# pfe-rs/lk-s-2022-estimacija-pokreta

Hardware: AMD Instinct MI355X
Metric: Mpix/s flow (1024x436, bcd_times=4) (higher is better)
Workload: dtype f64; 1 GPU; single 1024x436 Sintel-shape pair per step per GPU, forward only, bcd_times=4 (BASELINE.json configs[1]); cells 64x27, 150 labels/px; pairs_in_flight_per_gpu=7, mode=batch

## Files before the change

### include/dflow.h

```cpp
#ifndef DFLOW_H
#define DFLOW_H

#include <stddef.h>
#include <stdint.h>

#ifdef __cplusplus
extern "C" {
#endif

#define DFLOW_VERSION 1
#define DFLOW_DESC 68
#define DFLOW_MAX_LABELS 160

#define DFLOW_FLAG_KNN_EXACT 1

#define DFLOW_FLAG_DESCR_F16 8
#define DFLOW_DESC_PITCH_F16 72

#define DFLOW_OK 0
#define DFLOW_EINVAL (-1)
#define DFLOW_ENOSPC (-2)
#define DFLOW_EHIP (-3)

#define DFLOW_DP_SENTINEL 800000.0
// ... 4 lines not shown
    int32_t maxnprop;
    int32_t knn;
    int32_t window;
    int32_t ngauss;
    int32_t tpsi;
    int32_t max_attempts;
    float tphi;
    float sigma;
    double lamda;
    uint64_t seed;
    int32_t label_pitch;
    int32_t flags;
} dflow_params;

int dflow_version(void);
const char *dflow_last_error(void);

void dflow_default_params(dflow_params *p, int32_t pich, int32_t picw, int32_t cellh, int32_t cellw);

size_t dflow_workspace_bytes(const dflow_params *p);

int dflow_daisy(const dflow_params *p, const uint8_t *d_bgr, void *d_descr,
                void *d_ws, size_t ws_bytes, void *stream);

int dflow_knn_proposals(const dflow_params *p, const void *d_descr1, const void *d_descr2,
                        uint32_t *d_proposals, float *d_lcosts, int32_t *d_nprop, int32_t *d_bestlabels,
                        void *d_ws, size_t ws_bytes, void *stream);

int dflow_knn_proposals_timed(const dflow_params *p, const void *d_descr1, const void *d_descr2,
                              uint32_t *d_proposals, float *d_lcosts, int32_t *d_nprop, int32_t *d_bestlabels,
                              void *d_ws, size_t ws_bytes, void *stream, float *h_ms, double *h_mfma_issued);

#define DFLOW_KNN_STATS_N 13
int dflow_knn_screen_stats(const dflow_params *p, void *d_ws, size_t ws_bytes, void *stream, int64_t *h_stats);

#define DFLOW_KNN_STATS_ALL_N 14
int dflow_knn_screen_stats_n(const dflow_params *p, void *d_ws, size_t ws_bytes, void *stream, int64_t *h_stats, int n_stats);

int dflow_neighbour_proposals(const dflow_params *p, const void *d_descr1, const void *d_descr2,
                              uint32_t *d_proposals, float *d_lcosts, int32_t *d_nprop,
                              const int32_t *d_bestlabels, void *d_ws, size_t ws_bytes, void *stream);

int dflow_bcd_prepare(const dflow_params *p, const uint32_t *d_proposals, const float *d_lcosts, const int32_t *d_nprop,
                      void *d_ws, size_t ws_bytes, void *stream);

int dflow_bcd_phase(const dflow_params *p, const uint32_t *d_proposals, const int32_t *d_nprop,
// ... 74 lines not shown
```

### lk-s-2022-estimacija-pokreta_amd/_lib.py

```python
import ctypes as C
import os
import subprocess

_HERE = os.path.dirname(os.path.abspath(__file__))
CSRC = os.path.join(_HERE, "csrc")
LIB_PATH = os.path.join(CSRC, "libdflow.so")

FLAG_KNN_EXACT = 1
FLAG_DESCR_F16 = 8
DESC_PITCH_F16 = 72
VAR_FLAG_SOR_UNFUSED = 1
EVAL_UVV, EVAL_DYDX = 0, 1
EVAL_FLAG_ACCUMULATE = 1


class DflowError(RuntimeError):
    pass


class Params(C.Structure):
    _fields_ = [("pich", C.c_int32), ("picw", C.c_int32), ("cellh", C.c_int32), ("cellw", C.c_int32),
                ("maxnprop", C.c_int32), ("knn", C.c_int32), ("window", C.c_int32), ("ngauss", C.c_int32),
                ("tpsi", C.c_int32), ("max_attempts", C.c_int32), ("tphi", C.c_float), ("sigma", C.c_float),
                ("lamda", C.c_double), ("seed", C.c_uint64), ("label_pitch", C.c_int32), ("flags", C.c_int32)]


class VarParams(C.Structure):
    _fields_ = [("alpha", C.c_float), ("gamma", C.c_float), ("delta", C.c_float), ("sigma", C.c_float),
                ("sor_omega", C.c_float), ("niter_outer", C.c_int32), ("niter_inner", C.c_int32),
                ("niter_solver", C.c_int32), ("flags", C.c_uint32)]


class EvalStats(C.Structure):
    _fields_ = [("n", C.c_uint64), ("n_out_abs", C.c_uint64), ("n_out_kitti", C.c_uint64), ("n_nonfinite", C.c_uint64),
                ("n_gt_valid", C.c_uint64), ("n_test_valid", C.c_uint64), ("sum_err", C.c_double), ("max_err", C.c_float),
                ("reserved", C.c_uint32)]


_vp, _sz, _i32, _f32, _f64 = C.c_void_p, C.c_size_t, C.c_int32, C.c_float, C.c_double
_pp = C.POINTER(Params)
_SIGNATURES = {
    "dflow_version": (C.c_int, []),
    "dflow_last_error": (C.c_char_p, []),
    "dflow_default_params": (None, [_pp, _i32, _i32, _i32, _i32]),
    "dflow_workspace_bytes": (_sz, [_pp]),
    "dflow_daisy": (C.c_int, [_pp, _vp, _vp, _vp, _sz, _vp]),
    "dflow_knn_proposals": (C.c_int, [_pp, _vp, _vp, _vp, _vp, _vp, _vp, _vp, _sz, _vp]),
    "dflow_knn_proposals_timed": (C.c_int, [_pp, _vp, _vp, _vp, _vp, _vp, _vp, _vp, _sz, _vp, C.POINTER(_f32), C.POINTER(_f64)]),
    "dflow_knn_screen_stats": (C.c_int, [_pp, _vp, _sz, _vp, C.POINTER(C.c_int64)]),
    "dflow_knn_screen_stats_n": (C.c_int, [_pp, _vp, _sz, _vp, C.POINTER(C.c_int64), _i32]),
    "dflow_neighbour_proposals": (C.c_int, [_pp, _vp, _vp, _vp, _vp, _vp, _vp, _vp, _sz, _vp]),
    "dflow_bcd_prepare": (C.c_int, [_pp, _vp, _vp, _vp, _vp, _sz, _vp]),
    "dflow_bcd_phase": (C.c_int, [_pp, _vp, _vp, _vp, _i32, _vp, _sz, _vp]),
    "dflow_bcd_sweep": (C.c_int, [_pp, _vp, _vp, _vp, _vp, _sz, _vp]),
    "dflow_bcd_phase_batch": (C.c_int, [_pp, _i32, _vp, _vp, _i32, _vp, _sz, _vp]),
    "dflow_bcd_sweep_batch": (C.c_int, [_pp, _i32, _vp, _vp, _vp, _sz, _vp]),
    "dflow_labels_to_flow": (C.c_int, [_pp, _vp, _vp, _vp, _vp]),
    "dflow_fb_consistency": (C.c_int, [_pp, _vp, _vp, _f32, _vp, _vp]),
    "dflow_pack_compat": (C.c_int, [_pp, _vp, _vp, _vp, _vp]),
    "dflow_remove_small_segments_host": (C.c_int, [_vp, _i32, _i32, _f32, _i32]),
    "dflow_canny_workspace_bytes": (_sz, [_i32, _i32]),
    "dflow_canny_edges": (C.c_int, [_i32, _i32, _vp, _f64, _f64, _vp, _vp, _vp, _sz, _vp]),
    "dflow_pb_workspace_bytes": (_sz, [_i32, _i32]),
    "dflow_pb_edges": (C.c_int, [_i32, _i32, _vp, _i32, _vp, _vp, _vp, _sz, _vp]),
    "dflow_epic_workspace_bytes": (_sz, [_i32, _i32]),
    "dflow_epic_interpolate": (C.c_int, [_i32, _i32, _vp, _vp, _i32, _f64, _i32, _vp, _vp, _vp, _vp, _vp, _vp, _sz, _vp]),
    "dflow_epic_last_stats": (C.c_int, [_vp, _vp]),
    "dflow_epic_prefilter_workspace_bytes": (_sz, [_i32, _i32]),
    "dflow_epic_prefilter": (C.c_int, [_i32, _i32, _vp, _vp, _vp, _f64, _i32, _f64, _f64, _vp, _vp, _vp, _vp, _vp, _sz, _vp]),
# ... 67 lines not shown
```

### lk-s-2022-estimacija-pokreta_amd/csrc/abi.hip

```cpp
#include <math.h>
#include <stdarg.h>
#include <stdio.h>
#include <stdlib.h>
#include <string.h>
#include "dflow_common.h"

static thread_local char g_err[512] = "";

int dflow_set_error(int code, const char *fmt, ...)
{
    va_list ap;
    va_start(ap, fmt);
    vsnprintf(g_err, sizeof(g_err), fmt, ap);
    va_end(ap);
    return code;
}

int dflow_check_launch(const char *what)
{
    hipError_t e = hipGetLastError();
    if (e != hipSuccess) return dflow_set_error(DFLOW_EHIP, "%s: %s", what, hipGetErrorString(e));
    return DFLOW_OK;
}

// ... 26 lines not shown
    if (!(p->sigma > 0.0f) || p->sigma > 8.0f) return dflow_set_error(DFLOW_EINVAL, "sigma=%g outside (0,8]", (double)p->sigma);
    if (p->max_attempts < p->ngauss) return dflow_set_error(DFLOW_EINVAL, "max_attempts < ngauss");
    if (p->flags & ~(DFLOW_FLAG_KNN_EXACT | DFLOW_FLAG_DESCR_F16)) return dflow_set_error(DFLOW_EINVAL, "unknown flags 0x%x", (unsigned)p->flags);
    return DFLOW_OK;
}

extern "C" {

int dflow_version(void) { return DFLOW_VERSION; }

const char *dflow_last_error(void) { return g_err; }

void dflow_default_params(dflow_params *p, int32_t pich, int32_t picw, int32_t cellh, int32_t cellw)
{
    memset(p, 0, sizeof(*p));
    p->pich = pich; p->picw = picw; p->cellh = cellh; p->cellw = cellw;
    p->maxnprop = 150; p->knn = 5; p->window = 2; p->ngauss = 25; p->tpsi = 8; p->max_attempts = 1 << 16;
    p->tphi = 2.5f; p->sigma = 8.0f; p->lamda = 0.05; p->seed = 0; p->label_pitch = 160;
}

size_t dflow_workspace_bytes(const dflow_params *p)
{
    if (dflow_check_params(p) != DFLOW_OK) return 0;
    size_t m = daisy_ws_bytes(p);
    for (size_t b : {bcd_ws_bytes(p), neighbour_ws_bytes(p), knn_mfma_supported(p) ? knn_mfma_ws_bytes(p) : (size_t)0})
        if (b > m) m = b;
    return m + DFLOW_WS_SLACK;
}

#define CHECK_PTR(x) do { if (!(x)) return dflow_set_error(DFLOW_EINVAL, "%s: %s is NULL", __func__, #x); } while (0)
#define CHECK_WS(need) do { if (!d_ws || ws_bytes < (need)) \
    return dflow_set_error(DFLOW_ENOSPC, "%s: workspace %zu < %zu bytes", __func__, ws_bytes, (size_t)(need)); } while (0)

int dflow_daisy(const dflow_params *p, const uint8_t *d_bgr, void *d_descr, void *d_ws, size_t ws_bytes, void *stream)
{
    int rc = dflow_check_params(p); if (rc) return rc;
    CHECK_PTR(d_bgr); CHECK_PTR(d_descr); CHECK_WS(daisy_ws_bytes(p));
    return launch_daisy(p, d_bgr, d_descr, d_ws, (hipStream_t)stream);
}

int dflow_knn_proposals(const dflow_params *p, const void *d_descr1, const void *d_descr2, uint32_t *d_proposals,
                        float *d_lcosts, int32_t *d_nprop, int32_t *d_bestlabels, void *d_ws, size_t ws_bytes, void *stream)
{
    int rc = dflow_check_params(p); if (rc) return rc;
    CHECK_PTR(d_descr1); CHECK_PTR(d_descr2); CHECK_PTR(d_proposals); CHECK_PTR(d_lcosts); CHECK_PTR(d_nprop); CHECK_PTR(d_bestlabels);
    if ((p->flags & DFLOW_FLAG_KNN_EXACT) || !knn_mfma_supported(p))
        return launch_knn(p, d_descr1, d_descr2, d_proposals, d_lcosts, d_nprop, d_bestlabels, (hipStream_t)stream);
    CHECK_WS(knn_mfma_ws_bytes(p));
    return launch_knn_mfma(p, d_descr1, d_descr2, d_proposals, d_lcosts, d_nprop, d_bestlabels, d_ws, (hipStream_t)stream);
}

int dflow_knn_proposals_timed(const dflow_params *p, const void *d_descr1, const void *d_descr2, uint32_t *d_proposals,
                              float *d_lcosts, int32_t *d_nprop, int32_t *d_bestlabels, void *d_ws, size_t ws_bytes, void *stream,
                              float *h_ms, double *h_mfma_issued)
{
    int rc = dflow_check_params(p); if (rc) return rc;
    CHECK_PTR(d_descr1); CHECK_PTR(d_descr2); CHECK_PTR(d_proposals); CHECK_PTR(d_lcosts); CHECK_PTR(d_nprop); CHECK_PTR(d_bestlabels);
    CHECK_PTR(h_ms);
    if ((p->flags & DFLOW_FLAG_KNN_EXACT) || !knn_mfma_supported(p))
        return dflow_set_error(DFLOW_EINVAL, "%s: the MFMA-screened search does not run for these parameters", __func__);
    CHECK_WS(knn_mfma_ws_bytes(p));
// ... 281 lines not shown
```

### lk-s-2022-estimacija-pokreta_amd/csrc/daisy.hip

```cpp
#include <math.h>
#include "dflow_common.h"

#define MAX_TAPS 9
struct Taps { int n; float k[MAX_TAPS]; };

struct GridTab { double gy[17], gx[17]; };

__device__ static inline int clampi(int v, int lo, int hi) { return v < lo ? lo : (v > hi ? hi : v); }

__device__ static inline float gray_of(const uint8_t *__restrict__ bgr, int W, int y, int x)
{
    return (float)gray_u8(bgr, W, y, x) / 255.0f;
}

template <typename T> __device__ static inline T tmul(float k, T v);
template <> __device__ inline float tmul<float>(float k, float v) { return k * v; }
template <> __device__ inline float4 tmul<float4>(float k, float4 v) { return make_float4(k * v.x, k * v.y, k * v.z, k * v.w); }
__device__ static inline float tadd(float a, float b) { return a + b; }
__device__ static inline float4 tadd(float4 a, float4 b) { return make_float4(a.x + b.x, a.y + b.y, a.z + b.z, a.w + b.w); }

struct LayerW { float wc[4], ws[4]; };

#define FX 32
#define FY 8
__global__ void __launch_bounds__(FX * FY) front_kernel(const uint8_t *__restrict__ bgr, float4 *__restrict__ lay, int H, int W, Taps t, LayerW w)
{
    __shared__ float g[FY + 6][FX + 6], th[FY + 6][FX + 2], sm[FY + 2][FX + 2];
    const int gx0 = blockIdx.x * FX, gy0 = blockIdx.y * FY, tid = threadIdx.y * FX + threadIdx.x;
    for (int i = tid; i < (FY + 6) * (FX + 6); i += FX * FY) {
        const int r = i / (FX + 6), c = i % (FX + 6);
        g[r][c] = gray_of(bgr, W, clampi(gy0 - 3 + r, 0, H - 1), clampi(gx0 - 3 + c, 0, W - 1));
    }
    __syncthreads();
    for (int i = tid; i < (FY + 6) * (FX + 2); i += FX * FY) {
        const int r = i / (FX + 2), c = i % (FX + 2);
        const int X = clampi(gx0 - 1 + c, 0, W - 1);
        float acc = t.k[0] * g[r][clampi(X - 2, 0, W - 1) - (gx0 - 3)];
#pragma unroll
        for (int j = 1; j < 5; j++) acc = acc + t.k[j] * g[r][clampi(X - 2 + j, 0, W - 1) - (gx0 - 3)];
        th[r][c] = acc;
    }
    __syncthreads();
    for (int i = tid; i < (FY + 2) * (FX + 2); i += FX * FY) {
        const int r = i / (FX + 2), c = i % (FX + 2);
        const int Y = clampi(gy0 - 1 + r, 0, H - 1);
        float acc = t.k[0] * th[clampi(Y - 2, 0, H - 1) - (gy0 - 3)][c];
#pragma unroll
        for (int j = 1; j < 5; j++) acc = acc + t.k[j] * th[clampi(Y - 2 + j, 0, H - 1) - (gy0 - 3)][c];
        sm[r][c] = acc;
    }
    __syncthreads();
    const int x = gx0 + threadIdx.x, y = gy0 + threadIdx.y;
    if (x >= W || y >= H) return;
    const int c = threadIdx.x + 1, r = threadIdx.y + 1;
    const float dx = (sm[r][c + 1] - sm[r][c - 1]) * 0.5f;
    const float dy = (sm[r + 1][c] - sm[r - 1][c]) * 0.5f;
    float v[4];
#pragma unroll
    for (int l = 0; l < 4; l++) { float q = dx * w.wc[l] + dy * w.ws[l]; v[l] = q > 0.0f ? q : 0.0f; }
    lay[(size_t)y * W + x] = make_float4(v[0], v[1], v[2], v[3]);
}

#define BX 32
#define BY 16
#define BR 4
__global__ void __launch_bounds__(BX * BY / 2) blur2d_kernel(const float4 *__restrict__ src, float4 *__restrict__ dst, int H, int W, Taps t)
{
    __shared__ float4 s[BY + 2 * BR][BX + 2 * BR], h[BY + 2 * BR][BX];
    const int r = t.n / 2;
    const int gx0 = blockIdx.x * BX, gy0 = blockIdx.y * BY, tid = threadIdx.y * BX + threadIdx.x, nthr = BX * BY / 2;
    const int sw = BX + 2 * r, sh = BY + 2 * r;
    for (int i = tid; i < sh * sw; i += nthr) {
        const int rr = i / sw, cc = i % sw;
        s[rr][cc] = src[(size_t)clampi(gy0 - r + rr, 0, H - 1) * W + clampi(gx0 - r + cc, 0, W - 1)];
    }
    __syncthreads();
    for (int i = tid; i < sh * BX; i += nthr) {
        const int rr = i / BX, cc = i % BX;
        float4 acc = tmul<float4>(t.k[0], s[rr][cc]);
        for (int j = 1; j < t.n; j++) acc = tadd(acc, tmul<float4>(t.k[j], s[rr][cc + j]));
        h[rr][cc] = acc;
    }
    __syncthreads();
    const int x = gx0 + threadIdx.x;
    if (x >= W) return;
#pragma unroll
    for (int half = 0; half < 2; half++) {
        const int ly = threadIdx.y + half * (BY / 2), y = gy0 + ly;
        if (y >= H) break;
        float4 acc = tmul<float4>(t.k[0], h[ly][threadIdx.x]);
        for (int j = 1; j < t.n; j++) acc = tadd(acc, tmul<float4>(t.k[j], h[ly + j][threadIdx.x]));
        dst[(size_t)y * W + x] = acc;
    }
}

__global__ void gather_kernel(const float4 *__restrict__ cubes, float4 *__restrict__ descr, int H, int W, GridTab g, int f16)
{
    size_t gid = (size_t)blockIdx.x * blockDim.x + threadIdx.x;
    size_t total = (size_t)H * W * 17;
    if (gid >= total) return;
    int region = (int)(gid % 17);
    size_t pix = gid / 17;
    int y = (int)(pix / W), x = (int)(pix % W);
    int ring = region == 0 ? 0 : (region - 1) / 4;
    const float4 *cube = cubes + (size_t)ring * H * W;
    double yy = (double)y + g.gy[region], xx = (double)x + g.gx[region];
    float4 out = make_float4(0.f, 0.f, 0.f, 0.f);
    bool ok = true;
    if (region != 0) {
        float xf = (float)xx, yf = (float)yy;
        ok = (0.0f <= xf && xf < (float)(W - 1) && 0.0f <= yf && yf < (float)(H - 1));
    }
    int mnx = (int)xx, mny = (int)yy;
    if (ok && !(mnx >= W - 2 || mny >= H - 2)) {
        float4 A = cube[(size_t)mny * W + mnx], B = cube[(size_t)(mny + 1) * W + mnx];
        float4 C = cube[(size_t)mny * W + mnx + 1], D = cube[(size_t)(mny + 1) * W + mnx + 1];
        double alpha = mnx + 1 - xx, beta = mny + 1 - yy;
        float w0 = (float)(alpha * beta);
        float w1 = (float)(beta - w0);
        float w2 = (float)(alpha - w0);
// ... 17 lines not shown
{
    int fsz = (int)(5.0 * sigma);
    if (fsz % 2 == 0) fsz++;
    if (fsz < 3) fsz = 3;
    return fsz;
}

static Taps gaussian_taps(int n, double sigma)
{
    Taps t;
    t.n = n;
    double scale2x = -0.5 / (sigma * sigma), sum = 0.0;
    for (int i = 0; i < n; i++) {
        double x = i - (n - 1) * 0.5;
        t.k[i] = (float)exp(scale2x * x * x);
        sum += t.k[i];
    }
    sum = 1.0 / sum;
    for (int i = 0; i < n; i++) t.k[i] = (float)(t.k[i] * sum);
    for (int i = n; i < MAX_TAPS; i++) t.k[i] = 0.0f;
    return t;
}

struct DaisyWs { float4 *tmp, *lay, *cubes; size_t bytes; };
static DaisyWs daisy_ws(const dflow_params *p, void *ws)
{
    const size_t N = (size_t)p->pich * p->picw;
    WsCarver c(ws);
    float4 *tmp = c.take<float4>(N), *lay = c.take<float4>(N), *cubes = c.take<float4>(4 * N);
    return {tmp, lay, cubes, c.bytes};
}

size_t daisy_ws_bytes(const dflow_params *p) { return daisy_ws(p, nullptr).bytes; }

int launch_daisy(const dflow_params *p, const uint8_t *bgr, void *descr, void *ws, hipStream_t s)
{
    const double pi = 3.14159265358979323846;
    int H = p->pich, W = p->picw;
    size_t N = (size_t)H * W;
    const DaisyWs w = daisy_ws(p, ws);
    float4 *const tmp = w.tmp, *const lay = w.lay, *const cubes = w.cubes;
    dim3 blk(256);

    Taps t = gaussian_taps(5, 0.5);
    LayerW lw;
    for (int l = 0; l < 4; l++) {
        float angle = (float)(2 * l * pi / 4);
        lw.wc[l] = (float)cos((double)angle);
        lw.ws[l] = (float)sin((double)angle);
    }
    hipLaunchKernelGGL(front_kernel, dim3((W + FX - 1) / FX, (H + FY - 1) / FY), dim3(FX, FY), 0, s, bgr, lay, H, W, t, lw);
    dim3 bgrd((W + BX - 1) / BX, (H + BY - 1) / BY), bblk(BX, BY / 2);
    {
        double sg = sqrt(1.6 * 1.6 - 0.25);
        t = gaussian_taps(filter_size((float)sg), (float)sg);
        hipLaunchKernelGGL(blur2d_kernel, bgrd, bblk, 0, s, (const float4 *)lay, tmp, H, W, t);
    }
    double sig[4];
    for (int r = 0; r < 4; r++) sig[r] = (r + 1) * (5.0 / 4 / 2);
    const float4 *prev = tmp;
    for (int r = 0; r < 4; r++) {
        double sg = r == 0 ? sig[0] : sqrt(sig[r] * sig[r] - sig[r - 1] * sig[r - 1]);
        t = gaussian_taps(filter_size(sg), sg);
        hipLaunchKernelGGL(blur2d_kernel, bgrd, bblk, 0, s, prev, cubes + (size_t)r * N, H, W, t);
        prev = cubes + (size_t)r * N;
    }
    GridTab g;
    double r_step = 5.0 / 4.0, t_step = 2 * pi / 4;
    g.gy[0] = 0.0; g.gx[0] = 0.0;
    for (int r = 0; r < 4; r++)
        for (int a = 0; a < 4; a++) {
            g.gy[1 + r * 4 + a] = (r + 1) * r_step * sin(a * t_step);
            g.gx[1 + r * 4 + a] = (r + 1) * r_step * cos(a * t_step);
        }
    size_t total = N * 17;
    hipLaunchKernelGGL(gather_kernel, dim3((unsigned)((total + 255) / 256)), blk, 0, s, (const float4 *)cubes,
                       (float4 *)descr, H, W, g, (p->flags & DFLOW_FLAG_DESCR_F16) ? 1 : 0);
    return dflow_check_launch("daisy kernels");
}
```

### lk-s-2022-estimacija-pokreta_amd/csrc/dflow_common.h

```cpp
#pragma once
#include <hip/hip_runtime.h>
#include <stdint.h>
#include "../../include/dflow.h"

#define DFLOW_FILL_PROPOSAL 0xFFFFFFFFu
#define DFLOW_FILL_COST 1000.0f

struct Geom {
    int H, W, ch, cw, ncx, ncy, win;
    __host__ __device__ int cellx(int x) const { int c = x / cw; return c < ncx ? c : ncx - 1; }
    __host__ __device__ int celly(int y) const { int c = y / ch; return c < ncy ? c : ncy - 1; }
    __host__ __device__ int x0(int ci) const { return ci * cw; }
    __host__ __device__ int y0(int cj) const { return cj * ch; }
    __host__ __device__ int x1(int ci) const { return ci == ncx - 1 ? W : (ci + 1) * cw; }
    __host__ __device__ int y1(int cj) const { return cj == ncy - 1 ? H : (cj + 1) * ch; }
    struct Window {
        int imin, imax, jmin, jmax;
        __host__ __device__ int slot(int ci, int cj) const { return (ci - imin) * (jmax - jmin + 1) + (cj - jmin); }
    };
    __host__ __device__ Window window(int qci, int qcj) const
    {
        return {max(0, qci - win), min(ncx - 1, qci + win), max(0, qcj - win), min(ncy - 1, qcj + win)};
    }
};
// ... 139 lines not shown

template <typename T_> struct DescrType { using T = T_; static constexpr bool F16 = sizeof(T_) == 2; };
template <typename F> static inline void with_descr_type(const dflow_params *p, F &&f)
{
    if (descr_f16(p)) f(DescrType<_Float16>()); else f(DescrType<float>());
}

int dflow_set_error(int code, const char *fmt, ...);
int dflow_check_launch(const char *what);
int dflow_check_params(const dflow_params *p);
#define DFLOW_HIP(x) do { hipError_t e_ = (x); if (e_ != hipSuccess) return dflow_set_error(DFLOW_EHIP, "%s: %s", #x, hipGetErrorString(e_)); } while (0)

static inline size_t align256(size_t v) { return (v + 255) & ~(size_t)255; }
struct WsCarver {
    uintptr_t base;
    size_t bytes = 0;
    explicit WsCarver(void *ws) : base((uintptr_t)ws) {}
    template <typename T> T *take(size_t count) { T *r = (T *)(base + bytes); bytes = align256(bytes + count * sizeof(T)); return r; }
};
#define DFLOW_WS_SLACK 256

int launch_daisy(const dflow_params *p, const uint8_t *bgr, void *descr, void *ws, hipStream_t s);
size_t daisy_ws_bytes(const dflow_params *p);
int launch_knn(const dflow_params *p, const void *d1, const void *d2, uint32_t *proposals, float *lcosts,
               int32_t *nprop, int32_t *bestlabels, hipStream_t s);
#define KNN_MFMA_EVENTS 7
int launch_knn_fix(const dflow_params *p, const void *d1, const void *d2, uint32_t *proposals, float *lcosts,
                   const int *ovf_count, const int4 *ovf_list, int ovf_cap, const int *flags, hipStream_t s);
int launch_knn_mfma(const dflow_params *p, const void *d1, const void *d2, uint32_t *proposals, float *lcosts,
                    int32_t *nprop, int32_t *bestlabels, void *ws, hipStream_t s, hipEvent_t *ev = nullptr);
double knn_mfma_issued(const dflow_params *p);
int knn_mfma_stats(const dflow_params *p, void *ws, hipStream_t s, int64_t *h_out);
size_t knn_mfma_ws_bytes(const dflow_params *p);
bool knn_mfma_supported(const dflow_params *p);
int launch_neighbour(const dflow_params *p, const void *d1, const void *d2, uint32_t *proposals, float *lcosts,
                     int32_t *nprop, const int32_t *bestlabels, void *ws, hipStream_t s);
size_t neighbour_ws_bytes(const dflow_params *p);
int launch_bcd_phase(const dflow_params *p, const int32_t *nprop, int32_t *bestlabels, int phase, void *ws, hipStream_t s);
int launch_bcd_phase_batch(const dflow_params *p, int npass, const int32_t *const *nprop, int32_t *const *bestlabels, int phase,
                           void *const *ws, hipStream_t s);
size_t bcd_ws_bytes(const dflow_params *p);
int launch_bcd_prepare(const dflow_params *p, const uint32_t *proposals, const float *lcosts, const int32_t *nprop, void *ws,
                       hipStream_t s);
int launch_labels_to_flow(const dflow_params *p, const uint32_t *proposals, const int32_t *bestlabels, float *flow,
                          hipStream_t s);
int launch_pack_compat(const dflow_params *p, const uint32_t *proposals, const int32_t *nprop, uint8_t *packed, hipStream_t s);
// ... 27 lines not shown
```

### lk-s-2022-estimacija-pokreta_amd/csrc/knn.hip

```cpp
#include "dflow_common.h"

#define KNN_THREADS 256

struct KnnArgs {
    Geom g;
    int LP, chunks;
    float tphi;
};

struct Top5 {
    float d0, d1, d2, d3, d4;
    int i0, i1, i2, i3, i4;
};

template <typename T> __device__ static inline float canon_dist(const float (&q)[DFLOW_DESC], const T *__restrict__ c)
{
    float acc = 0.0f;
    if constexpr (sizeof(T) == 4) {
        const float4 *__restrict__ c4 = reinterpret_cast<const float4 *>(c);
#pragma unroll
        for (int k = 0; k < DFLOW_DESC / 4; k++) {
            float4 v = c4[k];
            float e;
            e = q[4 * k] - v.x; acc = __fmaf_rn(e, e, acc);
// ... 73 lines not shown
    desc_load_row(q, gd1, pix);
    const int cimin = max(0, qci - g.win), cimax = min(g.ncx - 1, qci + g.win);
    const int cjmin = max(0, qcj - g.win), cjmax = min(g.ncy - 1, qcj + g.win);
    float mind = 1000.0f;
    int bestl = 0, slot = 0;
    for (int ci = cimin; ci <= cimax; ci++)
        for (int cj = cjmin; cj <= cjmax; cj++) {
            Top5 t;
            search_cell_exact(q, gd2, g, ci, cj, t);
            float c[5];
            emit_cell(t, g, ci, cj, pix, qy, qx, slot, a.LP, a.tphi, active, gd1, gd2, gproposals, glcosts, c);
#pragma unroll
            for (int qq = 0; qq < 5; qq++)
                if (c[qq] < mind) { mind = c[qq]; bestl = slot + qq; }
            slot += 5;
        }
    if (active) {
        gnprop[pix] = slot;
        gbestlabels[pix] = bestl;
        for (int s = slot; s < a.LP; s++) { gproposals[pix * a.LP + s] = DFLOW_FILL_PROPOSAL; glcosts[pix * a.LP + s] = DFLOW_FILL_COST; }
    }
}

#define KNN_FIX_WAVES 16
#define KNN_FIX_CHUNK 64
#define KNN_FIX_BLOCKS 256
template <bool BY_INDEX> __device__ static inline void top5_place(Top5 &t, float cd, int cidx)
{
    bool sh = false;
    auto slot = [&](float &d, int &i) {
        if (sh || cd < d || (BY_INDEX && cd == d && cidx < i)) { const float td = d; const int ti = i; d = cd; i = cidx; cd = td; cidx = ti; sh = true; }
    };
    slot(t.d0, t.i0); slot(t.d1, t.i1); slot(t.d2, t.i2); slot(t.d3, t.i3); slot(t.d4, t.i4);
}
__device__ static inline void top5_insert(Top5 &t, float cd, int cidx) { top5_place<false>(t, cd, cidx); }
__device__ static inline void top5_merge(Top5 &t, float cd, int cidx) { top5_place<true>(t, cd, cidx); }

template <typename T>
__global__ void __launch_bounds__(64 * KNN_FIX_WAVES) knn_fix_kernel(KnnArgs a, const T *__restrict__ gd1, const T *__restrict__ gd2,
                                                        uint32_t *__restrict__ gproposals, float *__restrict__ glcosts,
                                                        const int *__restrict__ ovf_count, const int4 *__restrict__ ovf_list,
                                                        int ovf_cap, const int *__restrict__ flags, int qwaves)
{
    __shared__ float pd[KNN_FIX_WAVES][5][64];
    __shared__ int pi[KNN_FIX_WAVES][5][64];
    __shared__ __attribute__((aligned(16))) float cand[2][KNN_FIX_CHUNK][DFLOW_DESC_PITCH_H];
    const Geom g = a.g;
    const int win = 2 * g.win + 1;
    const int nov = *ovf_count;
    const bool all = (*flags != 0) || nov > ovf_cap;
    const int total = all ? g.ncx * g.ncy * qwaves * win * win : nov;
    const int lane = threadIdx.x & 63, wave = threadIdx.x >> 6;
    for (int item = blockIdx.x; item < total; item += gridDim.x) {
        int qcell, qstart, ci, cj;
        if (all) {
            int b = item;
            const int wslot = b % (win * win); b /= win * win;
            qstart = (b % qwaves) * 64; qcell = b / qwaves;
            const Geom::Window w = g.window(qcell % g.ncx, qcell / g.ncx);
            const int ncyw = w.jmax - w.jmin + 1;
            ci = w.imin + wslot / ncyw; cj = w.jmin + wslot % ncyw;
            if (ci > w.imax) continue;
// ... 120 lines not shown
```

### lk-s-2022-estimacija-pokreta_amd/csrc/knn_mfma.hip

```cpp
#include "dflow_common.h"
#include "knn_pca.h"
#include "row_stage.h"

typedef _Float16 half8 __attribute__((ext_vector_type(8)));
typedef float f32x16 __attribute__((ext_vector_type(16)));

#define KM_ALPHA 64.0f
#define KM_K 48
#define KM_KSTEPS (KM_K / 16)
#define KM_KD 40
#define KM_SLOT_N 40
#define KM_SLOT_QE 41
#define KM_SLOT_EN 42
#define KM_SLOT_H 43
#define KM_SLOT_S 45
#define KM_SLOT_ONE 46
#define KM_XSCALE 64.0
#define KM_SSCALE 4096.0
#define KM_NORM2_MAX 30000.0
#define KM_WAVES 8
#define KM_THREADS (64 * KM_WAVES)
#define KM_QPW 64
#define KM_QPB (KM_WAVES * KM_QPW)
#ifndef KM_CHUNK
// ... 40 lines not shown
    const int wl = g.x1(g.ncx - 1) - g.x0(g.ncx - 1), hl = g.y1(g.ncy - 1) - g.y0(g.ncy - 1);
    return km_cell_base(g, 0, g.ncy - 1) + (size_t)(g.ncx - 1) * km_pad(g.cw * hl) + km_pad(wl * hl);
}

__device__ static inline void km_store_sentinel(_Float16 *row)
{
    half8 *o = reinterpret_cast<half8 *>(row);
    const half8 z = {(_Float16)0.0f, (_Float16)0.0f, (_Float16)0.0f, (_Float16)0.0f, (_Float16)0.0f, (_Float16)0.0f, (_Float16)0.0f, (_Float16)0.0f};
    half8 t8 = z;
    t8[KM_SLOT_H - 40] = (_Float16)60000.0f;
#pragma unroll
    for (int k = 0; k < KM_K / 8; k++) o[k] = k == KM_K / 8 - 1 ? t8 : z;
}

__device__ static inline _Float16 km_f16_up(double v) { return (_Float16)(float)(v * 1.001 + 1e-7); }

#define KM_Q_ZERO 1.0f
#define KM_Q_BAD 2.0f
struct KmCellTop { uint32_t idx[5]; float cost[5]; };

#define KM_RHO 2.65e-5
typedef float km_f2p __attribute__((ext_vector_type(2)));
template <typename T>
__global__ void __launch_bounds__(256) knn_prep_kernel(const T *__restrict__ d, const float *__restrict__ vt, _Float16 *__restrict__ h,
                                                       float2 *__restrict__ qs, float2 *__restrict__ z0, uint8_t *__restrict__ zflag,
                                                       int *__restrict__ cell_bad, Geom g, int which)
{
    int pix;
    size_t orow;
    if (which == 0) {
        pix = blockIdx.x * blockDim.x + threadIdx.x;
        if (pix >= g.H * g.W) return;
        orow = (size_t)pix;
    } else {
        const int ci = blockIdx.y % g.ncx, cj = blockIdx.y / g.ncx;
        const int cx0 = g.x0(ci), cy0 = g.y0(cj), ccw = g.x1(ci) - cx0, cnpts = ccw * (g.y1(cj) - cy0);
        const int pos = blockIdx.x * blockDim.x + threadIdx.x;
        if (pos >= km_pad(cnpts)) return;
        orow = km_cell_base(g, ci, cj) + pos;
        const int idx = (pos & 31) * km_ntiles(cnpts) + (pos >> 5);
        if (idx >= cnpts) {
            km_store_sentinel(h + orow * KM_K);
            z0[orow] = make_float2(INFINITY, 0.0f);
            zflag[orow] = 0;
            return;
        }
        pix = (cy0 + idx / ccw) * g.W + cx0 + idx % ccw;
    }
    float x[DFLOW_DESC];
    desc_load_row(x, d, (size_t)pix);
    if (which == 1) {
        const float4 zero[DFLOW_DESC / 4] = {};
        const PairDist zd = pair_dist(x, zero);
        z0[orow] = make_float2(zd.l2, zd.l1());
    }
    double sxall = 0.0;
    bool bad = false;
#pragma unroll
    for (int k = 0; k < DFLOW_DESC; k++) {
        const float sc = KM_ALPHA * x[k];
// ... 30 lines not shown
    const double ypl = fmax(0.0, ry - KM_RHO * rx), ypu = ry + KM_RHO * rx;
    const double nd = sqrt(fmax(0.0, sxall * (1.0 + 1.1 * PCA_DELTA_MAX) - ypl * ypl));
    if (which == 0) {
        last[KM_SLOT_N - 40] = -km_f16_up(nd);
        last[KM_SLOT_QE - 40] = -km_f16_up(sqrt(ss) * (1.0 / KM_XSCALE));
        last[KM_SLOT_EN - 40] = -km_f16_up(en * KM_XSCALE);
        last[KM_SLOT_H - 40] = (_Float16)-1.0f; last[KM_SLOT_H + 1 - 40] = (_Float16)-1.0f;
        last[KM_SLOT_S - 40] = (_Float16)(float)(-1.0 / KM_SSCALE);
        last[KM_SLOT_ONE - 40] = (_Float16)0.0f; last[KM_SLOT_ONE + 1 - 40] = (_Float16)0.0f;
        qs[pix] = make_float2(bad ? KM_Q_BAD : zero ? KM_Q_ZERO : 0.0f, (float)(0.5 * sxall * (1.0 + 1.5 * PCA_DELTA_MAX) * 1.0000002));
    } else {
        const double hh = 0.5 * sxall;
        const _Float16 p1 = (_Float16)(float)hh;
        const _Float16 p2 = (_Float16)(float)(hh - (double)(float)p1);
        const double hres = fabs(hh - (double)(float)p1 - (double)(float)p2);
        const double scs = (KM_ETA * 1.001 * hh + 3e-6 * hh + hres) * 1.0004;
        last[KM_SLOT_N - 40] = km_f16_up(nd);
        last[KM_SLOT_QE - 40] = km_f16_up((en + KM_ETA * sqrt(ss)) * KM_XSCALE);
        last[KM_SLOT_EN - 40] = km_f16_up(ypu * (1.0 / KM_XSCALE));
        last[KM_SLOT_H - 40] = p1; last[KM_SLOT_H + 1 - 40] = p2;
        last[KM_SLOT_S - 40] = km_f16_up(scs * KM_SSCALE);
        last[KM_SLOT_ONE - 40] = (_Float16)1.0f; last[KM_SLOT_ONE + 1 - 40] = (_Float16)1.0f;
        zflag[orow] = zero ? 1 : 0;
        if (bad) cell_bad[blockIdx.y] = 1;
    }
    o[KM_K / 8 - 1] = last;
}

__global__ void __launch_bounds__(256) knn_cell_post_kernel(_Float16 *__restrict__ h2, const float2 *__restrict__ z0,
                                                            const uint8_t *__restrict__ zflag, KmCellTop *__restrict__ ztop, Geom g)
{
    __shared__ int wsum[4];
    __shared__ unsigned long long wmin[4];
    const int ci = blockIdx.x % g.ncx, cj = blockIdx.x / g.ncx;
    const int cnpts = (g.x1(ci) - g.x0(ci)) * (g.y1(cj) - g.y0(cj));
    const int npad = km_pad(cnpts), ntiles = km_ntiles(cnpts);
    const size_t base = km_cell_base(g, ci, cj);
    const int tid = threadIdx.x, lane = tid & 63, wave = tid >> 6;
    int running = 0;
    for (int c0 = 0; c0 < cnpts; c0 += 256) {
        const int idx = c0 + tid;
        const int pos = (idx % ntiles) * 32 + idx / ntiles;
        const bool z = idx < cnpts && zflag[base + pos] != 0;
        const unsigned long long bal = __ballot(z);
        if (lane == 0) wsum[wave] = __popcll(bal);
        __syncthreads();
        int before = running + __popcll(bal & ((1ull << lane) - 1ull));
// ... 682 lines not shown
    a.evrows = k.evrows;
    return a;
}

bool knn_mfma_supported(const dflow_params *p)
{
    Geom g = make_geom(p);
    return max_cell_points(g) <= KM_MAXPTS && p->window >= 0 && p->window <= 2;
}

#define KM_MARK(i) do { if (tev) DFLOW_HIP(hipEventRecord(tev[i], s)); } while (0)
int launch_knn_mfma(const dflow_params *p, const void *d1, const void *d2, uint32_t *proposals, float *lcosts,
                    int32_t *nprop, int32_t *bestlabels, void *ws, hipStream_t s, hipEvent_t *tev)
{
    Geom g = make_geom(p);
    const size_t N = (size_t)g.H * g.W;
    const KmWs k = km_ws(p, ws);
    DFLOW_HIP(hipMemsetAsync(k.ctr, 0, k.zero_bytes, s));
    int nb = (int)((N + 255) / 256);
    KM_MARK(0);
    int rc = launch_knn_pca(p, d2, k.vt, k.ctr + 1, k.pca_ws, s);
    if (rc) return rc;
    KM_MARK(1);
    const dim3 cgrid((km_pad(max_cell_points(g)) + 255) / 256, g.ncx * g.ncy);
    with_descr_type(p, [&](auto d) {
        using T = typename decltype(d)::T;
        hipLaunchKernelGGL(knn_prep_kernel<T>, dim3(nb), dim3(256), 0, s, (const T *)d1, (const float *)k.vt, k.h1, k.qs, (float2 *)nullptr, (uint8_t *)nullptr, (int *)nullptr, g, 0);
        hipLaunchKernelGGL(knn_prep_kernel<T>, cgrid, dim3(256), 0, s, (const T *)d2, (const float *)k.vt, k.h2, (float2 *)nullptr, k.z0, k.zflag, k.cell_bad, g, 1);
    });
    hipLaunchKernelGGL(knn_cell_post_kernel, dim3(g.ncx * g.ncy), dim3(256), 0, s, k.h2, (const float2 *)k.z0, (const uint8_t *)k.zflag, k.ztop, g);
    rc = dflow_check_launch("knn_cell_post_kernel");
    if (rc) return rc;

    KM_MARK(2);
    const KmGeom a = km_geom(p, k);
    int win = 2 * g.win + 1;
    int wgs_per_cell = (win * win * a.qwaves + KM_WAVES - 1) / KM_WAVES;
    KmScreen sc;
    sc.h1 = k.h1; sc.h2 = k.h2; sc.qs = k.qs; sc.cell_bad = k.cell_bad; sc.ev = k.ev; sc.ev_cnt = k.ev_cnt;
    size_t shmem = (size_t)KM_NBUF * KM_ABUF;
    hipLaunchKernelGGL(knn_screen_kernel, dim3(g.ncx * g.ncy * wgs_per_cell), dim3(KM_THREADS), shmem, s, a, sc);
    rc = dflow_check_launch("knn_screen_kernel");
    if (rc) return rc;
    KM_MARK(3);
    KmResolve rs;
    rs.d1 = d1; rs.d2 = d2; rs.ev = k.ev; rs.ev_cnt = k.ev_cnt; rs.qs = k.qs; rs.ztop = k.ztop; rs.proposals = proposals; rs.lcosts = lcosts;
    rs.ovf_count = k.ctr; rs.ovf_list = k.ovf; rs.ovf_cap = (int)k.nl;
    rs.heavy_count = k.ctr + 2; rs.heavy_list = k.heavy; rs.heavy_cap = KM_HEAVY_CAP;
    const dim3 rgrid((unsigned)(g.ncx * g.ncy * win * a.qwaves));
    with_descr_type(p, [&](auto d) { hipLaunchKernelGGL(knn_resolve_kernel<decltype(d)::F16>, rgrid, dim3(64), 0, s, a, rs); });
    rc = dflow_check_launch("knn_resolve_kernel");
// ... 107 lines not shown
```

### lk-s-2022-estimacija-pokreta_amd/pipeline.py

```python
import ctypes as C

import numpy as np
import torch

from . import _lib
from . import flowio

DEFAULT_CELLS = {
    (375, 1241): (25, 73),
    (375, 1242): (25, 54),
    (436, 1024): (27, 64),
}


def default_cells(pich, picw):
    if (pich, picw) in DEFAULT_CELLS:
        return DEFAULT_CELLS[(pich, picw)]
    return max(5, pich // 15), max(5, picw // 17)


class DiscreteFlow:

    def __init__(self, pich, picw, cellh=None, cellw=None, device="cuda:0", seed=0, **overrides):
        if not torch.cuda.is_available():
            raise _lib.DflowError("no HIP device visible: the dflow hot path has no CPU fallback")
        if cellh is None or cellw is None:
            cellh, cellw = default_cells(pich, picw)
        self.p = _lib.default_params(pich, picw, cellh, cellw, seed=seed, **overrides)
        self.ws_bytes = int(_lib.lib().dflow_workspace_bytes(C.byref(self.p)))
        _lib.check(0 if self.ws_bytes else -1, "dflow_workspace_bytes")
        self.device = torch.device(device)
        self._descr_f16 = bool(self.p.flags & _lib.FLAG_DESCR_F16)
        H, W, LP = pich, picw, self.p.label_pitch
        dev = self.device
        self.descrs1 = self._new_descr()
        self.descrs2 = self._new_descr()
        self.proposals = torch.empty((H, W, LP), dtype=torch.int32, device=dev)
        self.lcosts = torch.empty((H, W, LP), dtype=torch.float32, device=dev)
        self.nprop = torch.empty((H, W), dtype=torch.int32, device=dev)
        self.bestlabels = torch.empty((H, W), dtype=torch.int32, device=dev)
        self.flow = torch.empty((H, W, 2), dtype=torch.float32, device=dev)
        self.ws = torch.empty(self.ws_bytes, dtype=torch.uint8, device=dev)
        self._img = torch.empty((H, W, 3), dtype=torch.uint8, device=dev)
        self._bcd_ready = False

    @property
    def descr_f16(self):
        return self._descr_f16

    def _new_descr(self):
        H, W = self.p.pich, self.p.picw
        if self.descr_f16:
            return torch.zeros((H, W, _lib.DESC_PITCH_F16), dtype=torch.float16, device=self.device)
        return torch.empty((H, W, 68), dtype=torch.float32, device=self.device)

    def _stream(self):
        return _lib.stream(self.device)

    def _pp(self):
        if bool(self.p.flags & _lib.FLAG_DESCR_F16) != self._descr_f16:
            raise _lib.DflowError("DFLOW_FLAG_DESCR_F16 changed after construction: the descriptor planes are %s"
                                  % ("binary16 (H,W,72)" if self._descr_f16 else "float32 (H,W,68)"))
        return C.byref(self.p)

    def izracunajDaisy(self, picture, out=None):
        H, W = self.p.pich, self.p.picw
        if isinstance(picture, np.ndarray):
            if picture.shape != (H, W, 3) or picture.dtype != np.uint8:
                raise ValueError("picture must be uint8 (%d,%d,3)" % (H, W))
            self._img.copy_(torch.from_numpy(np.ascontiguousarray(picture)))
            img = self._img
        else:
            if tuple(picture.shape) != (H, W, 3) or picture.dtype != torch.uint8 or not picture.is_contiguous():
                raise ValueError("picture must be a contiguous uint8 (%d,%d,3) tensor" % (H, W))
            img = picture
        if out is None:
            out = self._new_descr()
        self._bcd_ready = False
        _lib.call("dflow_daisy", self._pp(), img.data_ptr(), out.data_ptr(), self.ws.data_ptr(), self.ws_bytes, self._stream())
        return out

    def load_pair(self, pic3, pic4):
        self.izracunajDaisy(pic3, out=self.descrs1)
        self.izracunajDaisy(pic4, out=self.descrs2)

    def set_descriptors(self, descrs1, descrs2):
        for dst, src in ((self.descrs1, descrs1), (self.descrs2, descrs2)):
            dst[..., :68].copy_(torch.as_tensor(src, dtype=torch.float32).to(dst.dtype))

    def descriptors_f32(self, which):
        return (self.descrs1, self.descrs2)[which][..., :68].to(torch.float32)

    def generisi(self):
        self._bcd_ready = False
        _lib.call("dflow_knn_proposals", self._pp(), self.descrs1.data_ptr(), self.descrs2.data_ptr(), self.proposals.data_ptr(),
                  self.lcosts.data_ptr(), self.nprop.data_ptr(), self.bestlabels.data_ptr(), self.ws.data_ptr(), self.ws_bytes,
                  self._stream())

    KNN_KERNELS = ("basis", "prep", "knn_screen_kernel", "knn_resolve_kernel", "knn_fix_kernel", "knn_finalize_kernel")

    def generisi_timed(self):
        self._bcd_ready = False
        ms = (C.c_float * 6)()
        issued = C.c_double()
        _lib.call("dflow_knn_proposals_timed", self._pp(), self.descrs1.data_ptr(), self.descrs2.data_ptr(), self.proposals.data_ptr(),
                  self.lcosts.data_ptr(), self.nprop.data_ptr(), self.bestlabels.data_ptr(), self.ws.data_ptr(), self.ws_bytes,
                  self._stream(), ms, C.byref(issued))
# ... 332 lines not shown
```

Baseline: 40.36 Mpix/s.

## Batch DAISY for both images and fuse KNN prep launches; retune knn_fix

Adds a paired DAISY path that runs front, blur and gather kernels once for both images through a grid z/y dimension, with a separate workspace per image. This halves the number of DAISY kernel launches and gives each launch a larger grid. The two knn_prep launches (query and candidate cells) are merged into one grid that picks its role from the block index. The knn_fix kernel also goes from 16 to 4 waves per block, with a smaller chunk and a min-blocks launch bound. The cost is a larger workspace, since the DAISY scratch buffers are now allocated twice.

```diff
diff --git a/include/dflow.h b/include/dflow.h
--- a/include/dflow.h
+++ b/include/dflow.h
@@ -50,6 +50,9 @@
 
 int dflow_daisy(const dflow_params *p, const uint8_t *d_bgr, void *d_descr,
                 void *d_ws, size_t ws_bytes, void *stream);
+
+int dflow_daisy_pair(const dflow_params *p, const uint8_t *d_bgr1, const uint8_t *d_bgr2, void *d_descr1, void *d_descr2,
+                     void *d_ws, size_t ws_bytes, void *stream);
 
 int dflow_knn_proposals(const dflow_params *p, const void *d_descr1, const void *d_descr2,
                         uint32_t *d_proposals, float *d_lcosts, int32_t *d_nprop, int32_t *d_bestlabels,
diff --git a/lk-s-2022-estimacija-pokreta_amd/_lib.py b/lk-s-2022-estimacija-pokreta_amd/_lib.py
--- a/lk-s-2022-estimacija-pokreta_amd/_lib.py
+++ b/lk-s-2022-estimacija-pokreta_amd/_lib.py
@@ -45,6 +45,7 @@
     "dflow_default_params": (None, [_pp, _i32, _i32, _i32, _i32]),
     "dflow_workspace_bytes": (_sz, [_pp]),
     "dflow_daisy": (C.c_int, [_pp, _vp, _vp, _vp, _sz, _vp]),
+    "dflow_daisy_pair": (C.c_int, [_pp, _vp, _vp, _vp, _vp, _vp, _sz, _vp]),
     "dflow_knn_proposals": (C.c_int, [_pp, _vp, _vp, _vp, _vp, _vp, _vp, _vp, _sz, _vp]),
     "dflow_knn_proposals_timed": (C.c_int, [_pp, _vp, _vp, _vp, _vp, _vp, _vp, _vp, _sz, _vp, C.POINTER(_f32), C.POINTER(_f64)]),
     "dflow_knn_screen_stats": (C.c_int, [_pp, _vp, _sz, _vp, C.POINTER(C.c_int64)]),
diff --git a/lk-s-2022-estimacija-pokreta_amd/csrc/abi.hip b/lk-s-2022-estimacija-pokreta_amd/csrc/abi.hip
--- a/lk-s-2022-estimacija-pokreta_amd/csrc/abi.hip
+++ b/lk-s-2022-estimacija-pokreta_amd/csrc/abi.hip
@@ -72,7 +72,7 @@
 size_t dflow_workspace_bytes(const dflow_params *p)
 {
     if (dflow_check_params(p) != DFLOW_OK) return 0;
-    size_t m = daisy_ws_bytes(p);
+    size_t m = daisy_pair_ws_bytes(p);
     for (size_t b : {bcd_ws_bytes(p), neighbour_ws_bytes(p), knn_mfma_supported(p) ? knn_mfma_ws_bytes(p) : (size_t)0})
         if (b > m) m = b;
     return m + DFLOW_WS_SLACK;
@@ -87,6 +87,15 @@
     int rc = dflow_check_params(p); if (rc) return rc;
     CHECK_PTR(d_bgr); CHECK_PTR(d_descr); CHECK_WS(daisy_ws_bytes(p));
     return launch_daisy(p, d_bgr, d_descr, d_ws, (hipStream_t)stream);
+}
+
+int dflow_daisy_pair(const dflow_params *p, const uint8_t *d_bgr1, const uint8_t *d_bgr2, void *d_descr1, void *d_descr2,
+                     void *d_ws, size_t ws_bytes, void *stream)
+{
+    int rc = dflow_check_params(p); if (rc) return rc;
+    CHECK_PTR(d_bgr1); CHECK_PTR(d_bgr2); CHECK_PTR(d_descr1); CHECK_PTR(d_descr2); CHECK_WS(daisy_pair_ws_bytes(p));
+    if (d_descr1 == d_descr2) return dflow_set_error(DFLOW_EINVAL, "%s: d_descr1 and d_descr2 are the same plane", __func__);
+    return launch_daisy_pair(p, d_bgr1, d_bgr2, d_descr1, d_descr2, d_ws, (hipStream_t)stream);
 }
 
 int dflow_knn_proposals(const dflow_params *p, const void *d_descr1, const void *d_descr2, uint32_t *d_proposals,
diff --git a/lk-s-2022-estimacija-pokreta_amd/csrc/daisy.hip b/lk-s-2022-estimacija-pokreta_amd/csrc/daisy.hip
--- a/lk-s-2022-estimacija-pokreta_amd/csrc/daisy.hip
+++ b/lk-s-2022-estimacija-pokreta_amd/csrc/daisy.hip
@@ -21,10 +21,17 @@
 
 struct LayerW { float wc[4], ws[4]; };
 
+template <typename T> struct PerImage {
+    T *p[2];
+    __device__ T *at(unsigned i) const { return i ? p[1] : p[0]; }
+};
+
 #define FX 32
 #define FY 8
-__global__ void __launch_bounds__(FX * FY) front_kernel(const uint8_t *__restrict__ bgr, float4 *__restrict__ lay, int H, int W, Taps t, LayerW w)
-{
+__global__ void __launch_bounds__(FX * FY) front_kernel(PerImage<const uint8_t> bgrs, PerImage<float4> lays, int H, int W, Taps t, LayerW w)
+{
+    const uint8_t *__restrict__ bgr = bgrs.at(blockIdx.z);
+    float4 *__restrict__ lay = lays.at(blockIdx.z);
     __shared__ float g[FY + 6][FX + 6], th[FY + 6][FX + 2], sm[FY + 2][FX + 2];
     const int gx0 = blockIdx.x * FX, gy0 = blockIdx.y * FY, tid = threadIdx.y * FX + threadIdx.x;
     for (int i = tid; i < (FY + 6) * (FX + 6); i += FX * FY) {
@@ -64,8 +71,10 @@
 #define BX 32
 #define BY 16
 #define BR 4
-__global__ void __launch_bounds__(BX * BY / 2) blur2d_kernel(const float4 *__restrict__ src, float4 *__restrict__ dst, int H, int W, Taps t)
-{
+__global__ void __launch_bounds__(BX * BY / 2) blur2d_kernel(PerImage<const float4> srcs, PerImage<float4> dsts, int H, int W, Taps t)
+{
+    const float4 *__restrict__ src = srcs.at(blockIdx.z);
+    float4 *__restrict__ dst = dsts.at(blockIdx.z);
     __shared__ float4 s[BY + 2 * BR][BX + 2 * BR], h[BY + 2 * BR][BX];
     const int r = t.n / 2;
     const int gx0 = blockIdx.x * BX, gy0 = blockIdx.y * BY, tid = threadIdx.y * BX + threadIdx.x, nthr = BX * BY / 2;
@@ -94,8 +103,10 @@
     }
 }
 
-__global__ void gather_kernel(const float4 *__restrict__ cubes, float4 *__restrict__ descr, int H, int W, GridTab g, int f16)
-{
+__global__ void gather_kernel(PerImage<const float4> cubess, PerImage<float4> descrs, int H, int W, GridTab g, int f16)
+{
+    const float4 *__restrict__ cubes = cubess.at(blockIdx.y);
+    float4 *__restrict__ descr = descrs.at(blockIdx.y);
     size_t gid = (size_t)blockIdx.x * blockDim.x + threadIdx.x;
     size_t total = (size_t)H * W * 17;
     if (gid >= total) return;
@@ -159,25 +170,33 @@
     return t;
 }
 
-struct DaisyWs { float4 *tmp, *lay, *cubes; size_t bytes; };
-static DaisyWs daisy_ws(const dflow_params *p, void *ws)
+struct DaisyWs { float4 *tmp[2], *lay[2], *cubes[2]; size_t bytes; };
+static DaisyWs daisy_ws(const dflow_params *p, void *ws, int nimg)
 {
     const size_t N = (size_t)p->pich * p->picw;
     WsCarver c(ws);
-    float4 *tmp = c.take<float4>(N), *lay = c.take<float4>(N), *cubes = c.take<float4>(4 * N);
-    return {tmp, lay, cubes, c.bytes};
-}
-
-size_t daisy_ws_bytes(const dflow_params *p) { return daisy_ws(p, nullptr).bytes; }
-
-int launch_daisy(const dflow_params *p, const uint8_t *bgr, void *descr, void *ws, hipStream_t s)
+    DaisyWs w = {};
+    for (int i = 0; i < nimg; i++) { w.tmp[i] = c.take<float4>(N); w.lay[i] = c.take<float4>(N); w.cubes[i] = c.take<float4>(4 * N); }
+    w.bytes = c.bytes;
+    return w;
+}
+
+size_t daisy_ws_bytes(const dflow_params *p) { return daisy_ws(p, nullptr, 1).bytes; }
+size_t daisy_pair_ws_bytes(const dflow_params *p) { return daisy_ws(p, nullptr, 2).bytes; }
+
+static int daisy_launches(const dflow_params *p, int nimg, const uint8_t *const *bgr, void *const *descr, void *ws, hipStream_t s)
 {
     const double pi = 3.14159265358979323846;
     int H = p->pich, W = p->picw;
     size_t N = (size_t)H * W;
-    const DaisyWs w = daisy_ws(p, ws);
-    float4 *const tmp = w.tmp, *const lay = w.lay, *const cubes = w.cubes;
+    const DaisyWs w = daisy_ws(p, ws, nimg);
+    const unsigned Z = (unsigned)nimg;
     dim3 blk(256);
+    PerImage<const uint8_t> in = {{bgr[0], nimg > 1 ? bgr[1] : nullptr}};
+    PerImage<float4> out = {{(float4 *)descr[0], nimg > 1 ? (float4 *)descr[1] : nullptr}};
+    PerImage<float4> lay = {{w.lay[0], w.lay[1]}}, tmp = {{w.tmp[0], w.tmp[1]}};
+    auto cube = [&](int r) { return PerImage<float4>{{w.cubes[0] + (size_t)r * N, nimg > 1 ? w.cubes[1] + (size_t)r * N : nullptr}}; };
+    auto ro = [](const PerImage<float4> &a) { return PerImage<const float4>{{a.p[0], a.p[1]}}; };
 
     Taps t = gaussian_taps(5, 0.5);
     LayerW lw;
@@ -186,21 +205,21 @@
         lw.wc[l] = (float)cos((double)angle);
         lw.ws[l] = (float)sin((double)angle);
     }
-    hipLaunchKernelGGL(front_kernel, dim3((W + FX - 1) / FX, (H + FY - 1) / FY), dim3(FX, FY), 0, s, bgr, lay, H, W, t, lw);
-    dim3 bgrd((W + BX - 1) / BX, (H + BY - 1) / BY), bblk(BX, BY / 2);
+    hipLaunchKernelGGL(front_kernel, dim3((W + FX - 1) / FX, (H + FY - 1) / FY, Z), dim3(FX, FY), 0, s, in, lay, H, W, t, lw);
+    dim3 bgrd((W + BX - 1) / BX, (H + BY - 1) / BY, Z), bblk(BX, BY / 2);
     {
         double sg = sqrt(1.6 * 1.6 - 0.25);
         t = gaussian_taps(filter_size((float)sg), (float)sg);
-        hipLaunchKernelGGL(blur2d_kernel, bgrd, bblk, 0, s, (const float4 *)lay, tmp, H, W, t);
+        hipLaunchKernelGGL(blur2d_kernel, bgrd, bblk, 0, s, ro(lay), tmp, H, W, t);
     }
     double sig[4];
     for (int r = 0; r < 4; r++) sig[r] = (r + 1) * (5.0 / 4 / 2);
-    const float4 *prev = tmp;
+    PerImage<const float4> prev = ro(tmp);
     for (int r = 0; r < 4; r++) {
         double sg = r == 0 ? sig[0] : sqrt(sig[r] * sig[r] - sig[r - 1] * sig[r - 1]);
         t = gaussian_taps(filter_size(sg), sg);
-        hipLaunchKernelGGL(blur2d_kernel, bgrd, bblk, 0, s, prev, cubes + (size_t)r * N, H, W, t);
-        prev = cubes + (size_t)r * N;
+        hipLaunchKernelGGL(blur2d_kernel, bgrd, bblk, 0, s, prev, cube(r), H, W, t);
+        prev = ro(cube(r));
     }
     GridTab g;
     double r_step = 5.0 / 4.0, t_step = 2 * pi / 4;
@@ -211,7 +230,20 @@
             g.gx[1 + r * 4 + a] = (r + 1) * r_step * cos(a * t_step);
         }
     size_t total = N * 17;
-    hipLaunchKernelGGL(gather_kernel, dim3((unsigned)((total + 255) / 256)), blk, 0, s, (const float4 *)cubes,
-                       (float4 *)descr, H, W, g, (p->flags & DFLOW_FLAG_DESCR_F16) ? 1 : 0);
+    hipLaunchKernelGGL(gather_kernel, dim3((unsigned)((total + 255) / 256), Z), blk, 0, s, ro(cube(0)), out, H, W, g,
+                       (p->flags & DFLOW_FLAG_DESCR_F16) ? 1 : 0);
     return dflow_check_launch("daisy kernels");
 }
+
+int launch_daisy(const dflow_params *p, const uint8_t *bgr, void *descr, void *ws, hipStream_t s)
+{
+    return daisy_launches(p, 1, &bgr, &descr, ws, s);
+}
+
+int launch_daisy_pair(const dflow_params *p, const uint8_t *bgr1, const uint8_t *bgr2, void *descr1, void *descr2, void *ws,
+                      hipStream_t s)
+{
+    const uint8_t *const bgr[2] = {bgr1, bgr2};
+    void *const descr[2] = {descr1, descr2};
+    return daisy_launches(p, 2, bgr, descr, ws, s);
+}
diff --git a/lk-s-2022-estimacija-pokreta_amd/csrc/dflow_common.h b/lk-s-2022-estimacija-pokreta_amd/csrc/dflow_common.h
--- a/lk-s-2022-estimacija-pokreta_amd/csrc/dflow_common.h
+++ b/lk-s-2022-estimacija-pokreta_amd/csrc/dflow_common.h
@@ -185,6 +185,9 @@
 
 int launch_daisy(const dflow_params *p, const uint8_t *bgr, void *descr, void *ws, hipStream_t s);
 size_t daisy_ws_bytes(const dflow_params *p);
+int launch_daisy_pair(const dflow_params *p, const uint8_t *bgr1, const uint8_t *bgr2, void *descr1, void *descr2, void *ws,
+                      hipStream_t s);
+size_t daisy_pair_ws_bytes(const dflow_params *p);
 int launch_knn(const dflow_params *p, const void *d1, const void *d2, uint32_t *proposals, float *lcosts,
                int32_t *nprop, int32_t *bestlabels, hipStream_t s);
 #define KNN_MFMA_EVENTS 7
diff --git a/lk-s-2022-estimacija-pokreta_amd/csrc/knn.hip b/lk-s-2022-estimacija-pokreta_amd/csrc/knn.hip
--- a/lk-s-2022-estimacija-pokreta_amd/csrc/knn.hip
+++ b/lk-s-2022-estimacija-pokreta_amd/csrc/knn.hip
@@ -119,8 +119,8 @@
     }
 }
 
-#define KNN_FIX_WAVES 16
-#define KNN_FIX_CHUNK 64
+#define KNN_FIX_WAVES 4
+#define KNN_FIX_CHUNK 28
 #define KNN_FIX_BLOCKS 256
 template <bool BY_INDEX> __device__ static inline void top5_place(Top5 &t, float cd, int cidx)
 {
@@ -134,7 +134,7 @@
 __device__ static inline void top5_merge(Top5 &t, float cd, int cidx) { top5_place<true>(t, cd, cidx); }
 
 template <typename T>
-__global__ void __launch_bounds__(64 * KNN_FIX_WAVES) knn_fix_kernel(KnnArgs a, const T *__restrict__ gd1, const T *__restrict__ gd2,
+__global__ void __launch_bounds__(64 * KNN_FIX_WAVES, 4) knn_fix_kernel(KnnArgs a, const T *__restrict__ gd1, const T *__restrict__ gd2,
                                                         uint32_t *__restrict__ gproposals, float *__restrict__ glcosts,
                                                         const int *__restrict__ ovf_count, const int4 *__restrict__ ovf_list,
                                                         int ovf_cap, const int *__restrict__ flags, int qwaves)
diff --git a/lk-s-2022-estimacija-pokreta_amd/csrc/knn_mfma.hip b/lk-s-2022-estimacija-pokreta_amd/csrc/knn_mfma.hip
--- a/lk-s-2022-estimacija-pokreta_amd/csrc/knn_mfma.hip
+++ b/lk-s-2022-estimacija-pokreta_amd/csrc/knn_mfma.hip
@@ -86,10 +86,15 @@
 #define KM_RHO 2.65e-5
 typedef float km_f2p __attribute__((ext_vector_type(2)));
 template <typename T>
-__global__ void __launch_bounds__(256) knn_prep_kernel(const T *__restrict__ d, const float *__restrict__ vt, _Float16 *__restrict__ h,
+__global__ void __launch_bounds__(256) knn_prep_kernel(const T *__restrict__ d1, const T *__restrict__ d2, const float *__restrict__ vt,
+                                                       _Float16 *__restrict__ h1, _Float16 *__restrict__ h2,
                                                        float2 *__restrict__ qs, float2 *__restrict__ z0, uint8_t *__restrict__ zflag,
-                                                       int *__restrict__ cell_bad, Geom g, int which)
-{
+                                                       int *__restrict__ cell_bad, Geom g, int qblocks, int cblocks)
+{
+    const int which = (int)blockIdx.x >= qblocks ? 1 : 0;
+    const T *__restrict__ d = which ? d2 : d1;
+    _Float16 *__restrict__ h = which ? h2 : h1;
+    const int cell = which ? ((int)blockIdx.x - qblocks) / cblocks : 0;
     int pix;
     size_t orow;
     if (which == 0) {
@@ -97,9 +102,9 @@
         if (pix >= g.H * g.W) return;
         orow = (size_t)pix;
     } else {
-        const int ci = blockIdx.y % g.ncx, cj = blockIdx.y / g.ncx;
+        const int ci = cell % g.ncx, cj = cell / g.ncx;
         const int cx0 = g.x0(ci), cy0 = g.y0(cj), ccw = g.x1(ci) - cx0, cnpts = ccw * (g.y1(cj) - cy0);
-        const int pos = blockIdx.x * blockDim.x + threadIdx.x;
+        const int pos = (((int)blockIdx.x - qblocks) % cblocks) * blockDim.x + threadIdx.x;
         if (pos >= km_pad(cnpts)) return;
         orow = km_cell_base(g, ci, cj) + pos;
         const int idx = (pos & 31) * km_ntiles(cnpts) + (pos >> 5);
@@ -176,7 +181,7 @@
         last[KM_SLOT_S - 40] = km_f16_up(scs * KM_SSCALE);
         last[KM_SLOT_ONE - 40] = (_Float16)1.0f; last[KM_SLOT_ONE + 1 - 40] = (_Float16)1.0f;
         zflag[orow] = zero ? 1 : 0;
-        if (bad) cell_bad[blockIdx.y] = 1;
+        if (bad) cell_bad[cell] = 1;
     }
     o[KM_K / 8 - 1] = last;
 }
@@ -905,11 +910,11 @@
     int rc = launch_knn_pca(p, d2, k.vt, k.ctr + 1, k.pca_ws, s);
     if (rc) return rc;
     KM_MARK(1);
-    const dim3 cgrid((km_pad(max_cell_points(g)) + 255) / 256, g.ncx * g.ncy);
+    const int cblocks = (km_pad(max_cell_points(g)) + 255) / 256;
     with_descr_type(p, [&](auto d) {
         using T = typename decltype(d)::T;
-        hipLaunchKernelGGL(knn_prep_kernel<T>, dim3(nb), dim3(256), 0, s, (const T *)d1, (const float *)k.vt, k.h1, k.qs, (float2 *)nullptr, (uint8_t *)nullptr, (int *)nullptr, g, 0);
-        hipLaunchKernelGGL(knn_prep_kernel<T>, cgrid, dim3(256), 0, s, (const T *)d2, (const float *)k.vt, k.h2, (float2 *)nullptr, k.z0, k.zflag, k.cell_bad, g, 1);
+        hipLaunchKernelGGL(knn_prep_kernel<T>, dim3(nb + cblocks * g.ncx * g.ncy), dim3(256), 0, s, (const T *)d1, (const T *)d2, (const float *)k.vt,
+                           k.h1, k.h2, k.qs, k.z0, k.zflag, k.cell_bad, g, nb, cblocks);
     });
     hipLaunchKernelGGL(knn_cell_post_kernel, dim3(g.ncx * g.ncy), dim3(256), 0, s, k.h2, (const float2 *)k.z0, (const uint8_t *)k.zflag, k.ztop, g);
     rc = dflow_check_launch("knn_cell_post_kernel");
diff --git a/lk-s-2022-estimacija-pokreta_amd/pipeline.py b/lk-s-2022-estimacija-pokreta_amd/pipeline.py
--- a/lk-s-2022-estimacija-pokreta_amd/pipeline.py
+++ b/lk-s-2022-estimacija-pokreta_amd/pipeline.py
@@ -42,6 +42,7 @@
         self.flow = torch.empty((H, W, 2), dtype=torch.float32, device=dev)
         self.ws = torch.empty(self.ws_bytes, dtype=torch.uint8, device=dev)
         self._img = torch.empty((H, W, 3), dtype=torch.uint8, device=dev)
+        self._img2 = torch.empty((H, W, 3), dtype=torch.uint8, device=dev)
         self._bcd_ready = False
 
     @property
@@ -63,17 +64,19 @@
                                   % ("binary16 (H,W,72)" if self._descr_f16 else "float32 (H,W,68)"))
         return C.byref(self.p)
 
-    def izracunajDaisy(self, picture, out=None):
+    def _device_image(self, picture, staging):
         H, W = self.p.pich, self.p.picw
         if isinstance(picture, np.ndarray):
             if picture.shape != (H, W, 3) or picture.dtype != np.uint8:
                 raise ValueError("picture must be uint8 (%d,%d,3)" % (H, W))
-            self._img.copy_(torch.from_numpy(np.ascontiguousarray(picture)))
-            img = self._img
-        else:
-            if tuple(picture.shape) != (H, W, 3) or picture.dtype != torch.uint8 or not picture.is_contiguous():
-                raise ValueError("picture must be a contiguous uint8 (%d,%d,3) tensor" % (H, W))
-            img = picture
+            staging.copy_(torch.from_numpy(np.ascontiguousarray(picture)))
+            return staging
+        if tuple(picture.shape) != (H, W, 3) or picture.dtype != torch.uint8 or not picture.is_contiguous():
+            raise ValueError("picture must be a contiguous uint8 (%d,%d,3) tensor" % (H, W))
+        return picture
+
+    def izracunajDaisy(self, picture, out=None):
+        img = self._device_image(picture, self._img)
         if out is None:
             out = self._new_descr()
         self._bcd_ready = False
@@ -81,8 +84,10 @@
         return out
 
     def load_pair(self, pic3, pic4):
-        self.izracunajDaisy(pic3, out=self.descrs1)
-        self.izracunajDaisy(pic4, out=self.descrs2)
+        img1, img2 = self._device_image(pic3, self._img), self._device_image(pic4, self._img2)
+        self._bcd_ready = False
+        _lib.call("dflow_daisy_pair", self._pp(), img1.data_ptr(), img2.data_ptr(), self.descrs1.data_ptr(), self.descrs2.data_ptr(),
+                  self.ws.data_ptr(), self.ws_bytes, self._stream())
 
     def set_descriptors(self, descrs1, descrs2):
         for dst, src in ((self.descrs1, descrs1), (self.descrs2, descrs2)):
```

Measured after the change: 40.89 Mpix/s (median of 6 runs). 1.3% higher.
